# harman097/RoboRugby

Hardware: AMD Instinct MI355X
Metric: env_steps_per_sec (higher is better)
Workload: dtype f64

## Files before the change

roborugby_amd/build.py:

```python
import hashlib
import os
import re
import shutil
import subprocess

HERE = os.path.dirname(os.path.abspath(__file__))
SRC = os.path.join(HERE, "csrc", "rr_kernels.hip")
SRC_KSTEP = os.path.join(HERE, "csrc", "rr_kstep_inst.hip")
SRC_DQN = os.path.join(HERE, "csrc", "rr_dqn.hip")
HDR_KSTEP = os.path.join(HERE, "csrc", "rr_kstep.hpp")
DEPS = [SRC, SRC_KSTEP, SRC_DQN, HDR_KSTEP, os.path.join(HERE, "csrc", "rr_sim.hpp"),
        os.path.join(HERE, "csrc", "rr_extras.hpp"), os.path.join(HERE, "csrc", "rr_hive.hpp"), os.path.join(HERE, "csrc", "rr_render.hpp"),
        os.path.join(os.path.dirname(HERE), "include", "roborugby_amd.h")]
LIB = os.path.join(HERE, "libroborugby_amd.so")
LIB_EXACT = os.path.join(HERE, "libroborugby_amd_exact.so")
HIPCC_FLAGS = ["-O3", "--offload-arch=gfx950", "-std=c++17", "-ffp-contract=off", "-fPIC", "-shared"]


def header_config_rows():
    with open(HDR_KSTEP) as f:
        text = f.read()
    parts = int(re.search(r"^#define RR_KSTEP_PARTS (\d+)$", text, re.M).group(1))
    table = re.search(r"^#else // the product library.*?^#endif", text, re.M | re.S).group(0)
    rows = [tuple(int(v) for v in m.groups()) for m in re.finditer(r"X\((\d+), (\d+), (\d+), (\d+), (\d+), (\d+), \w+, (\d+)\)", table)]
    if not rows or sorted({r[1] for r in rows}) != list(range(parts)):
        raise RuntimeError("csrc/rr_kstep.hpp: the configuration table does not use every part 0..RR_KSTEP_PARTS-1")
    return parts, rows


def header_config_table():
    parts, rows = header_config_rows()
    return parts, {r[2:6] for r in rows}


KSTEP_PARTS = 4
BUILT_SHAPES = {(1, 0, 1, 0), (2, 2, 4, 4), (1, 1, 1, 1)}


def find_hipcc():
    for cand in (shutil.which("hipcc"), "/opt/rocm/bin/hipcc"):
        if cand and os.path.exists(cand):
            return cand
    raise RuntimeError("hipcc not found: the MI355X library cannot be built here")


def sources_present():
    return all(os.path.exists(d) for d in DEPS)


def source_hash():
    h = hashlib.sha256(" ".join(HIPCC_FLAGS).encode())
    for d in DEPS:
        with open(d, "rb") as f:
            h.update(os.path.basename(d).encode() + b"\0" + f.read())
    return h.hexdigest()


def is_stale(exact=False):
    lib = LIB_EXACT if exact else LIB
    if not os.path.exists(lib) or not os.path.exists(lib + ".srchash"):
        return True
    with open(lib + ".srchash") as f:
        return f.read().strip() != source_hash()


def build_hip_library(force=False, verbose=False, jobs=None, exact=False):
    lib_path = LIB_EXACT if exact else LIB
    if not force and not is_stale(exact):
        return lib_path
    import tempfile
    from concurrent.futures import ThreadPoolExecutor
    if header_config_table() != (KSTEP_PARTS, BUILT_SHAPES):
        raise RuntimeError("roborugby_amd/build.py: KSTEP_PARTS / BUILT_SHAPES differ from the table in csrc/rr_kstep.hpp")
    digest = source_hash()
    hipcc = find_hipcc()
    cflags = [f for f in HIPCC_FLAGS if f != "-shared"] + (["-DRR_EXACT_TRIG=1"] if exact else [])
    jobs = jobs or int(os.environ.get("RR_BUILD_JOBS", "0")) or min(8, os.cpu_count() or 1)
    with tempfile.TemporaryDirectory(prefix="rr_build_") as tmpd:
        units = [(SRC, ["-DRR_SPLIT_BUILD"], os.path.join(tmpd, "rr_kernels.o"))]
        units += [(SRC_KSTEP, [f"-DRR_PART={k}"], os.path.join(tmpd, f"rr_kstep_{k}.o")) for k in range(KSTEP_PARTS)]
        units += [(SRC_DQN, [], os.path.join(tmpd, "rr_dqn.o"))]

        def compile_one(u):
            src, defs, obj = u
            cmd = [hipcc] + cflags + defs + ["-c", "-o", obj, src]
            if verbose:
                print(" ".join(cmd), flush=True)
            subprocess.check_call(cmd)
            return obj

        with ThreadPoolExecutor(max_workers=jobs) as ex:
            objs = list(ex.map(compile_one, units))
        tmp = lib_path + f".tmp{os.getpid()}"
        cmd = [hipcc, "--offload-arch=gfx950", "-fPIC", "-shared", "-o", tmp] + objs
# ... 66 lines not shown
```

roborugby_amd/csrc/rr_kernels.hip:

```cpp
#include <hip/hip_runtime.h>
#include <stdio.h>
#include <string.h>
#include <cmath>
#include <new>
#include <string>
#include <type_traits>
#include <cstdlib>

#include "../../include/roborugby_amd.h"
#include "rr_sim.hpp"
#include "rr_extras.hpp"
#include "rr_hive.hpp"
#include "rr_render.hpp"
#include "rr_kstep.hpp"

using namespace rr;


#ifndef RR_ORDER_SHIFT
#define RR_ORDER_SHIFT 2
#endif
constexpr int ORDER_BINS = 1024, ORDER_THREADS = 1024;
__global__ __launch_bounds__(ORDER_THREADS) void k_order(const uint32_t *cost, uint32_t *order, int ngroups) {
    __shared__ uint32_t hist[ORDER_BINS];
    for (int i = threadIdx.x; i < ORDER_BINS; i += ORDER_THREADS) hist[i] = 0;
    __syncthreads();
    for (int g = threadIdx.x; g < ngroups; g += ORDER_THREADS) {
        uint32_t c = cost[g] >> RR_ORDER_SHIFT;
        c = c > ORDER_BINS - 1 ? ORDER_BINS - 1 : c;
        atomicAdd(&hist[ORDER_BINS - 1 - c], 1u);
    }
    __syncthreads();
    __shared__ uint32_t scan[ORDER_BINS];
    uint32_t v = hist[threadIdx.x];
    scan[threadIdx.x] = v;
    __syncthreads();
    for (int off = 1; off < ORDER_BINS; off <<= 1) {
        uint32_t add = threadIdx.x >= (unsigned)off ? scan[threadIdx.x - off] : 0u;
        __syncthreads();
        scan[threadIdx.x] += add;
        __syncthreads();
    }
    hist[threadIdx.x] = scan[threadIdx.x] - v;
    __syncthreads();
    for (int g = threadIdx.x; g < ngroups; g += ORDER_THREADS) {
        uint32_t c = cost[g] >> RR_ORDER_SHIFT;
        c = c > ORDER_BINS - 1 ? ORDER_BINS - 1 : c;
        order[atomicAdd(&hist[ORDER_BINS - 1 - c], 1u)] = (uint32_t)g;
    }
}
__global__ void k_iota(uint32_t *order, int n) {
    int i = blockIdx.x * blockDim.x + threadIdx.x;
    if (i < n) order[i] = (uint32_t)i;
}

template <class C, typename O>
__global__ __launch_bounds__(64 * WAVES_PER_BLOCK) void k_reset(SimParams<typename C::Real> sp, typename C::Store *recs,
                                                               int32_t *irecs, int n, const uint8_t *mask, int init,
                                                               O *obs, O *obs_g) {
    using R = typename C::Real;
    __shared__ Arena<C> lds[arenas_per_block<C>()];
    const int wave = threadIdx.x / C::VW;
    const int arena = blockIdx.x * arenas_per_block<C>() + wave;
    if (arena >= n || wave >= arenas_per_block<C>()) return;
    Arena<C> &A = lds[wave];
    typename C::Store *rec = recs + (size_t)arena * Arena<C>::P_STRIDE;
    int32_t *irec = irecs + (size_t)arena * Arena<C>::I_STRIDE;
    int st = 0;
    if (init) {
        const int lane = threadIdx.x & (C::VW - 1);
        R *p = reinterpret_cast<R *>(&A.p);
        int32_t *q = reinterpret_cast<int32_t *>(&A.i);
        for (int k = lane; k < Arena<C>::P_REALS; k += C::VW) p[k] = (R)0;
        for (int k = lane; k < Arena<C>::I_INTS; k += C::VW) q[k] = 0;
        RR_SYNC();
        if (lane < C::NR) robot_set_clean_lane(A, sp, lane, (R)0, (R)0, lane < C::NRH ? (R)90 : (R)-90);
        if (lane < C::NB) ball_set_clean_lane(A, lane, (R)0, (R)0, (R)0, (R)0);
        if (lane == 0) A.i.episode = -1;
        RR_SYNC();
    } else {
        load_record(A, rec, irec);
    }
    const bool doit = init || !mask || mask[arena];
    if (doit) reset_arena(A, sp, sp.arena_offset + (uint64_t)arena, (uint64_t)(uint32_t)(A.i.episode + 1), st);
    else derive(A, sp);
    if (obs && doit) observe<C, O>(A, sp, 1, -1, -1, obs + (size_t)arena * 11, st);
    if (obs_g && doit) {
        if (!observe<C, O>(A, sp, -1, -1, -1, obs_g + (size_t)arena * 11, st)) {
            for (int k = threadIdx.x & (C::VW - 1); k < 11; k += C::VW) obs_g[(size_t)arena * 11 + k] = (O)NAN;
        }
    }
    store_record(A, rec, irec);
}

template <class C, typename O>
__global__ __launch_bounds__(64 * WAVES_PER_BLOCK) void k_observe(SimParams<typename C::Real> sp, const typename C::Store *recs,
                                                                 const int32_t *irecs, int n, int team, int ridx, int bidx,
                                                                 O *obs) {
    __shared__ Arena<C> lds[arenas_per_block<C>()];
    const int wave = threadIdx.x / C::VW;
    const int arena = blockIdx.x * arenas_per_block<C>() + wave;
    if (arena >= n || wave >= arenas_per_block<C>()) return;
    Arena<C> &A = lds[wave];
    load_record(A, recs + (size_t)arena * Arena<C>::P_STRIDE, irecs + (size_t)arena * Arena<C>::I_STRIDE);
    derive(A, sp);
    int st = 0;
    if (!observe<C, O>(A, sp, team, ridx, bidx, obs + (size_t)arena * 11, st)) {
        for (int k = threadIdx.x & (C::VW - 1); k < 11; k += C::VW) obs[(size_t)arena * 11 + k] = (O)NAN;
    }
}

template <class C>
__global__ void k_set_state(typename C::Store *recs, int32_t *irecs, int n, const double *robots, const int32_t *ri,
                            const double *balls, const int32_t *step) {
    using R = typename C::Real;
    int a = blockIdx.x * blockDim.x + threadIdx.x;
    if (a >= n) return;
    typename C::Store *rec = recs + (size_t)a * Arena<C>::P_STRIDE;
    int32_t *irec = irecs + (size_t)a * Arena<C>::I_STRIDE;
    using L = RecLayout<C>;
    constexpr int NR = C::NR, NB = C::NB;
    for (int r = 0; r < NR; r++) {
        for (int f = 0; f < L::ROBOT_FIELDS; f++) rec[L::robot_field(f) + r] = (typename C::Store)robots[((size_t)a * NR + r) * L::ROBOT_FIELDS + f];
        for (int f = 0; f < 3; f++) irec[L::robot_int(f) + r] = ri[((size_t)a * NR + r) * 3 + f];
    }
    for (int b = 0; b < NB; b++)
        for (int f = 0; f < L::BALL_FIELDS; f++) rec[L::ball_field(f) + b] = (typename C::Store)balls[((size_t)a * NB + b) * L::BALL_FIELDS + f];
    irec[L::STEP] = step[a];
    irec[L::FAULT] = 0;
// ... 158 lines not shown
    __shared__ Arena<C> lds[arenas_per_block<C>()];
    const int wave = threadIdx.x / C::VW;
    const int arena = blockIdx.x * arenas_per_block<C>() + wave;
    if (arena >= n || wave >= arenas_per_block<C>()) return;
    const int32_t *irec = irecs + (size_t)arena * Arena<C>::I_STRIDE;
    if constexpr (HELD) {
        if (hive_hold<C>(irec, held + arena)) return;
    }
    Arena<C> &A = lds[wave];
    const typename C::Store *rec = recs + (size_t)arena * Arena<C>::P_STRIDE;
    load_record(A, rec, irec);
    if (KIND == OBS_V2) derive(A, sp);
    Rec<C> q = { rec };
    hive_observe<C, O, KIND>(A, q, sp, robot_mask, assign + (size_t)arena * C::NR, obs + (size_t)arena * C::NR * 11);
}
__global__ __launch_bounds__(256) void k_hive_commit(int n, int nr, uint32_t robot_mask, const int32_t *fresh, const int32_t *assign,
                                                     const uint8_t *held, int32_t *accepted, float *thrust) {
    const int cell = blockIdx.x * 256 + threadIdx.x;
    if (cell >= n * nr) return;
    const int a = cell / nr, r = cell - a * nr;
    const size_t row = (size_t)a * nr;
    hive_commit(robot_mask, r, fresh + row, assign + row, held[a], accepted + row, thrust + 2 * row);
}
template <class C, typename O, int KIND, bool HELD = false>
__global__ __launch_bounds__(64 * WAVES_PER_BLOCK, lds_waves_per_simd<C>()) void k_hive_transition(
    SimParams<typename C::Real> sp, const typename C::Store *recs, const int32_t *irecs, int n, const typename C::Real *xs, uint32_t robot_mask,
    const int32_t *assign, const int32_t *status, const uint8_t *done, O *next_obs, O *reward, uint8_t *terminal, uint8_t *valid) {
    __shared__ Arena<C> lds[arenas_per_block<C>()];
    const int wave = threadIdx.x / C::VW;
    const int arena = blockIdx.x * arenas_per_block<C>() + wave;
    if (arena >= n || wave >= arenas_per_block<C>()) return;
    const size_t row = (size_t)arena * C::NR;
    if constexpr (HELD) {
        if (hive_idle<C, O>(status[arena], next_obs + row * 11, reward + row, terminal + row, valid + row)) return;
    }
    Arena<C> &A = lds[wave];
    const typename C::Store *rec = recs + (size_t)arena * Arena<C>::P_STRIDE;
    load_record(A, rec, irecs + (size_t)arena * Arena<C>::I_STRIDE);
    if (KIND == OBS_V2) derive(A, sp);
    Rec<C> q = { rec };
    hive_transition<C, O, KIND>(A, q, sp, xs + (size_t)arena * xs_stride<C>(), robot_mask, assign + row, status[arena], done[arena],
                                next_obs + row * 11, reward + row, terminal + row, valid + row);
}

__global__ void k_policy_chase(const float *obs, int n, int na, uint32_t noise_u32, uint64_t seed, uint64_t arena_offset,
                               const int32_t *step_of, uint32_t step, int32_t *actions) {
    const int a = blockIdx.x * blockDim.x + threadIdx.x;
    if (a >= n) return;
    const float d = fmodf(obs[(size_t)a * 11 + 1] - obs[(size_t)a * 11 + 0] + 540.0f, 360.0f) - 180.0f;
    int act = fabsf(d) < 8.0f ? 0 : (d > 0.0f ? 2 : 3);
    const uint64_t gid = arena_offset + (uint64_t)a;
    const uint32_t st = step_of ? (uint32_t)step_of[a] : step;
    uint32_t c[4] = { (uint32_t)gid, (uint32_t)(gid >> 32), st, 0x70C1u };
    philox4x32(c, (uint32_t)seed, (uint32_t)(seed >> 32));
    if (c[0] < noise_u32) act = (int)(c[1] & 7u);
    actions[(size_t)a * na] = act;
    for (int k = 1; k < na; k++) actions[(size_t)a * na + k] = (int)((c[2 + (k & 1)] >> (4 * (k >> 1))) & 7u);
}

typedef unsigned int u32x4 __attribute__((ext_vector_type(4)));
__global__ __launch_bounds__(256) void k_copy16(const u32x4 *__restrict__ src, u32x4 *__restrict__ dst, size_t n16) {
    const size_t i = (size_t)blockIdx.x * 256 + threadIdx.x;
    if (i < n16) dst[i] = src[i];
}

struct rr_env {
    rr_config cfg;
    int kind;
    int vw;
    void *recs;
    int32_t *irecs;
    size_t rec_bytes, irec_bytes;
    uint32_t *snap;
    int32_t *isnap;
    SimParams<double> spd;
    SimParams<float> spf;
    Program prog;
    bool custom_prog;
    bool track_prior;
    int32_t *gs;
    void *xs;
    int32_t *status_buf;
    uint32_t *order;
    uint32_t *cost;
    int ngroups;
    uint32_t *park;
    uint32_t budget;
    int32_t *flag;
};

static thread_local std::string g_err;
static int fail(int code, const std::string &msg) { g_err = msg; return code; }
#define HIP_TRY(expr)                                                                            \
    do {                                                                                         \
        hipError_t e_ = (expr);                                                                  \
        if (e_ != hipSuccess) return fail(-2, std::string(#expr) + ": " + hipGetErrorString(e_)); \
    } while (0)

template <typename R> static void fill_params(SimParams<R> &sp, const rr_config &c) {
    derive_constants(sp, c.arena_w, c.arena_h);
    sp.game_len = c.game_len_steps; sp.game_mode = c.game_mode; sp.time_limit = c.time_limit; sp.auto_reset = c.auto_reset;
    sp.reset_on_fault = c.reset_on_fault;
    sp.acc_external = 0;
    { const char *nm = getenv("RR_NO_MEMO"); sp.memo = (nm && atoi(nm)) ? 0 : 1; }
    sp.seed = c.seed; sp.arena_offset = c.arena_offset;
}
template <typename R> static const SimParams<R> &params_of(const rr_env *e);
template <> const SimParams<double> &params_of<double>(const rr_env *e) { return e->spd; }
template <> const SimParams<float> &params_of<float>(const rr_env *e) { return e->spf; }

template <class F> static int dispatch(const rr_env *e, F &&f) {
#define X(kind_, part_, a, b, c, d, R_, vw_) \
    if (e->kind == kind_) return f(Cfg<a, b, c, d, R_, vw_>{});
    RR_CFG_TABLE(X)
#undef X
    return fail(-1, "corrupt handle");
}
struct DeviceGuard {
    int prev = -1;
    bool switched = false;
    explicit DeviceGuard(int want) {
        if (hipGetDevice(&prev) == hipSuccess && prev != want) switched = (hipSetDevice(want) == hipSuccess);
    }
    ~DeviceGuard() { if (switched) (void)hipSetDevice(prev); }
};

template <class C> struct Typed {
    using Cfg = C;
    using R = typename C::Real;
    const rr_env *e;
    hipStream_t s;
    int n() const { return e->cfg.num_envs; }
    typename C::Store *recs() const { return static_cast<typename C::Store *>(e->recs); }
    int32_t *irecs() const { return e->irecs; }
    R *xs() const { return static_cast<R *>(e->xs); }
    const SimParams<R> &sp() const { return params_of<R>(e); }
    template <class... P, class... A> void per_thread(void (*k)(P...), const A &...a) const {
        hipLaunchKernelGGL(k, dim3((unsigned)((n() + 127) / 128)), dim3(128), 0, s, static_cast<P>(a)...);
    }
    template <class... P, class... A> void per_wave(void (*k)(P...), const A &...a) const {
        hipLaunchKernelGGL(k, dim3((unsigned)((n() + arenas_per_block<C>() - 1) / arenas_per_block<C>())), dim3(64 * WAVES_PER_BLOCK), 0, s,
                           static_cast<P>(a)...);
    }
};
template <typename O = float, class F>
static int on_handle(rr_env *e, const char *who, void *stream, F &&f, const char *f64_refusal = nullptr) {
    if (!e) return fail(-1, std::string(who) + ": null handle");
    DeviceGuard guard(e->cfg.device);
    int rc = dispatch(e, [&](auto c) {
        using C = decltype(c);
        if constexpr (std::is_same<O, double>::value && !std::is_same<typename C::Real, double>::value) return fail(-1, f64_refusal);
        else return f(Typed<C>{ e, (hipStream_t)stream });
    });
    if (rc) return rc;
    HIP_TRY(hipGetLastError());
    return 0;
}

extern "C" {

int rr_abi_version(void) { return RR_ABI_VERSION; }
int rr_exact_trig(void) { return RR_EXACT_TRIG; }
const char *rr_last_error(void) { return g_err.c_str(); }

int rr_create(const rr_config *cfg, rr_env **out) {
    if (!cfg || !out) return fail(-1, "rr_create: null argument");
    if (cfg->struct_size != (int32_t)sizeof(rr_config)) return fail(-1, "rr_create: rr_config.struct_size mismatch");
    if (cfg->num_envs <= 0) return fail(-1, "rr_create: num_envs must be positive");
    int shape = -1;
#define X(kind_, part_, a, b, c, d, R_, vw_) \
    if (shape < 0 && cfg->nr_happy == a && cfg->nr_grumpy == b && cfg->nb_pos == c && cfg->nb_neg == d) shape = kind_ % RR_NUM_SHAPES;
    RR_CFG_TABLE(X)
#undef X
#if defined(RR_CUSTOM_SHAPE)
    if (shape < 0) return fail(-1, "rr_create: this library was built for one shape only (roborugby_amd.build.build_shape_library) and it is not this one");
    if (cfg->dtype == RR_DTYPE_F32) return fail(-1, "rr_create: a one-shape library is built for RR_DTYPE_F64 and RR_DTYPE_F32_STATE only");
#else
    if (shape < 0)
        return fail(-1, "rr_create: unsupported entity counts (built shapes: 1+0 robots/1+0 balls, 2+2 robots/4+4 balls, 1+1 robots/1+1 balls; "
                        "any other counts: a one-shape library, roborugby_amd.build.build_shape_library / BatchedRoboRugbyEnv does it on demand)");
#endif
    if (cfg->dtype != RR_DTYPE_F64 && cfg->dtype != RR_DTYPE_F32 && cfg->dtype != RR_DTYPE_F32_STATE) return fail(-1, "rr_create: bad dtype");
    if (cfg->dtype == RR_DTYPE_F32_STATE && cfg->step_budget_clocks) return fail(-1, "rr_create: no step budget with RR_DTYPE_F32_STATE");
    if (!(cfg->arena_w >= 300 && cfg->arena_h >= 300 && cfg->arena_w <= 8192 && cfg->arena_h <= 8192))
        return fail(-1, "rr_create: arena size out of range [300, 8192]");
    if (cfg->game_len_steps <= 0) return fail(-1, "rr_create: game_len_steps must be positive");
    int ndev = 0;
    HIP_TRY(hipGetDeviceCount(&ndev));
    if (cfg->device < 0 || cfg->device >= ndev) return fail(-1, "rr_create: no such HIP device");
    DeviceGuard guard(cfg->device);
    rr_env *e = new (std::nothrow) rr_env();
    if (!e) return fail(-3, "rr_create: out of host memory");
    e->cfg = *cfg;
    e->kind = shape + RR_NUM_SHAPES * cfg->dtype;
    e->prog.n = 3; e->prog.id[0] = KEEPER_NAUGHTY; e->prog.id[1] = KEEPER_CHASE; e->prog.id[2] = KEEPER_PUSHPOS;
    fill_params(e->spd, *cfg);
    fill_params(e->spf, *cfg);
    size_t pstride = 0, preals = 0, snapw = 0, isnapw = 0;
    int apb = 1;
    const size_t rsz = cfg->dtype == RR_DTYPE_F64 ? 8 : 4;
    dispatch(e, [&](auto c) {
        using CC = decltype(c);
        e->vw = CC::VW;
        pstride = Arena<CC>::P_STRIDE; preals = Arena<CC>::P_REALS; snapw = Arena<CC>::SNAP_WORDS; isnapw = Arena<CC>::ISNAP_WORDS;
        apb = arenas_per_block<CC>();
        return 0;
    });
    const int n = cfg->num_envs;
    e->rec_bytes = pstride * rsz;
    e->irec_bytes = 0;
    hipError_t he = hipMalloc(&e->recs, e->rec_bytes * (size_t)n);
    if (he == hipSuccess && e->spd.memo) {
        he = hipMalloc((void **)&e->snap, 4 * snapw * (size_t)n);
        if (he == hipSuccess) he = hipMalloc((void **)&e->isnap, 4 * isnapw * (size_t)n);
    }
    if (he != hipSuccess) {
        rr_destroy(e);
        return fail(-3, std::string("rr_create: hipMalloc: ") + hipGetErrorString(he));
    }
    e->irecs = reinterpret_cast<int32_t *>(static_cast<char *>(e->recs) + preals * rsz);
    const int ng = (n + apb - 1) / apb;
    const char *no = getenv("RR_NO_ORDER");
    if (ng > 2048 && ng <= 65536 && !(no && atoi(no))) {
        if (hipMalloc((void **)&e->order, sizeof(uint32_t) * ng) == hipSuccess && hipMalloc((void **)&e->cost, sizeof(uint32_t) * ng) == hipSuccess) {
            e->ngroups = ng;
            hipLaunchKernelGGL(k_iota, dim3((ng + 255) / 256), dim3(256), 0, 0, e->order, ng);
            (void)hipMemset(e->cost, 0, sizeof(uint32_t) * ng);
        } else {
            if (e->order) (void)hipFree(e->order);
            e->order = nullptr; e->cost = nullptr;
        }
    }
    dispatch(e, [&](auto c) {
        Typed<decltype(c)> v = { e, nullptr };
        v.per_wave(k_reset<decltype(c), float>, v.sp(), v.recs(), v.irecs(), n, nullptr, 1, nullptr, nullptr);
        return 0;
    });
    he = hipGetLastError();
    if (he == hipSuccess) he = hipDeviceSynchronize();
    if (he != hipSuccess) {
        rr_destroy(e);
        return fail(-2, std::string("rr_create: init kernel: ") + hipGetErrorString(he));
    }
    if (cfg->step_budget_clocks) {
        if (int rc = rr_set_step_budget(e, cfg->step_budget_clocks)) { rr_destroy(e); return rc; }
    }
    *out = e;
    return 0;
}

int rr_destroy(rr_env *e) {
    if (!e) return 0;
    DeviceGuard guard(e->cfg.device);
    for (void *p : { e->recs, (void *)e->snap, (void *)e->isnap, e->xs, (void *)e->gs, (void *)e->status_buf, (void *)e->order, (void *)e->cost,
                     (void *)e->park, (void *)e->flag })
        if (p) (void)hipFree(p);
    delete e;
    return 0;
}

int rr_reset(rr_env *e, const uint8_t *mask, float *obs, float *obs_g, void *stream) {
    return on_handle(e, "rr_reset", stream, [&](auto v) {
        using C = typename decltype(v)::Cfg;
        v.per_wave(k_reset<C, float>, v.sp(), v.recs(), v.irecs(), v.n(), mask, 0, obs, obs_g);
        if (e->track_prior && e->xs)
            v.per_thread(k_extras_begin<C>, v.recs(), v.n(), v.xs(), mask);
        if (e->gs) v.per_thread(k_goal_clear<C>, v.n(), e->gs, mask);
        return 0;
    });
}

static int check_step_args(rr_env *e, const void *act, int32_t na, const void *obs, const void *reward, const void *done) {
    if (!e) return fail(-1, "rr_step: null handle");
    if (!act || !obs || !reward || !done) return fail(-1, "rr_step: actions/obs/reward/done must be non-null");
    const int nr = e->cfg.nr_happy + e->cfg.nr_grumpy;
    if (na < 0 || na > nr)
        return fail(-1, "rr_step: more actions than robots");
    return 0;
}

extern "C++" {
template <typename O>
static int step_impl(rr_env *e, const int32_t *actions, const float *thrust, int32_t na, O *obs, O *reward, uint8_t *done,
                     O *obs_g, O *reward_g, int32_t *status, void *stream, int nsteps = 1, int repeat = 0) {
    if ((e->custom_prog || e->track_prior || e->gs) && !status) status = e->status_buf;
    return on_handle<O>(e, "rr_step", stream, [&](auto v) {
        using C = typename decltype(v)::Cfg;
        const int n = v.n();
        const bool extras = e->custom_prog || e->track_prior;
        auto step = [&](auto kernel, int ns, int rep, uint32_t *park, uint32_t budget) {
            v.per_wave(kernel, v.sp(), v.recs(), v.irecs(), n, actions, thrust, na, obs, reward, done, obs_g, reward_g, status, e->order, e->cost,
                       ns, rep, e->snap, e->isnap, park, budget);
        };
        if (extras) v.per_thread(k_extras_begin<C>, v.recs(), n, v.xs(), nullptr);
        if constexpr (C::MIXED) {
            if (nsteps != 1 || e->park) return fail(-1, "RR_DTYPE_F32_STATE: rr_step only (no rr_rollout, no step budget)");
            step(k_step<C, O, false>, 1, 0, nullptr, 0);
        } else {
            if (nsteps == 1 && e->park) step(k_step<C, O, false, true>, 1, 0, e->park, e->budget);
            else if (nsteps == 1) step(k_step<C, O, false>, 1, 0, nullptr, 0);
            else if constexpr (std::is_same<O, float>::value) step(k_step<C, O, true>, nsteps, repeat, nullptr, 0);
            else return fail(-1, "rr_rollout: float outputs only");
        }
        if (e->order) hipLaunchKernelGGL(k_order, dim3(1), dim3(ORDER_THREADS), 0, v.s, (const uint32_t *)e->cost, e->order, e->ngroups);
        if (extras) v.per_thread(k_extras_end<C, O>, v.sp(), v.recs(), n, v.xs(), e->prog, e->custom_prog ? 1 : 0, reward, reward_g, status, done);
        if (e->gs) {
            int bd = 0;
            for (int k = 0; k < e->prog.n; k++) bd |= e->prog.id[k] == KEEPER_BASEDESTRUCTION;
            v.per_thread(k_goal<C, O>, v.sp(), v.recs(), v.irecs(), n, e->gs, bd, reward, reward_g, done, status);
        }
        return 0;
    }, "fp64 outputs need a handle created with RR_DTYPE_F64");
}
}

int rr_step(rr_env *e, const int32_t *actions, int32_t na, float *obs, float *reward, uint8_t *done, float *obs_g,
            float *reward_g, int32_t *status, void *stream) {
    if (int rc = check_step_args(e, actions, na, obs, reward, done)) return rc;
    return step_impl<float>(e, actions, nullptr, na, obs, reward, done, obs_g, reward_g, status, stream);
}
int rr_rollout(rr_env *e, const int32_t *actions, int32_t na, int32_t nsteps, int32_t repeat, float *obs, float *reward,
               uint8_t *done, float *obs_g, float *reward_g, int32_t *status, void *stream) {
    if (int rc = check_step_args(e, actions, na, obs, reward, done)) return rc;
    if (nsteps < 1 || nsteps > 4096) return fail(-1, "rr_rollout: nsteps must be in 1..4096");
    if (e->custom_prog || e->track_prior || e->gs)
        return fail(-1, "rr_rollout: the side kernels of a custom reward program / prior-step tracking / goal scoring bracket single steps; use rr_step");
    if (e->park) return fail(-1, "rr_rollout: not on a handle that has had a step budget (arenas may be parked mid-step); use rr_step");
    return step_impl<float>(e, actions, nullptr, na, obs, reward, done, obs_g, reward_g, status, stream, (int)nsteps, repeat != 0);
}
int rr_step_thrust(rr_env *e, const float *thrust, int32_t nk, float *obs, float *reward, uint8_t *done, float *obs_g,
                   float *reward_g, int32_t *status, void *stream) {
    if (int rc = check_step_args(e, thrust, nk, obs, reward, done)) return rc;
    return step_impl<float>(e, nullptr, thrust, nk, obs, reward, done, obs_g, reward_g, status, stream);
}
int rr_step_f64(rr_env *e, const int32_t *actions, int32_t na, double *obs, double *reward, uint8_t *done, double *obs_g,
                double *reward_g, int32_t *status, void *stream) {
    if (int rc = check_step_args(e, actions, na, obs, reward, done)) return rc;
    return step_impl<double>(e, actions, nullptr, na, obs, reward, done, obs_g, reward_g, status, stream);
}
int rr_step_thrust_f64(rr_env *e, const float *thrust, int32_t nk, double *obs, double *reward, uint8_t *done, double *obs_g,
                       double *reward_g, int32_t *status, void *stream) {
    if (int rc = check_step_args(e, thrust, nk, obs, reward, done)) return rc;
    return step_impl<double>(e, nullptr, thrust, nk, obs, reward, done, obs_g, reward_g, status, stream);
}

static int ensure_snapshot_buffer(rr_env *e) {
    if (e->xs) return 0;
    size_t bytes = 0;
    dispatch(e, [&](auto c) { using C = decltype(c); bytes = sizeof(typename C::Real) * xs_stride<C>() * (size_t)e->cfg.num_envs; return 0; });
    HIP_TRY(hipMalloc(&e->xs, bytes));
    HIP_TRY(hipMemset(e->xs, 0, bytes));
    return 0;
}
static int ensure_status_buffer(rr_env *e) {
    if (!e->status_buf) HIP_TRY(hipMalloc((void **)&e->status_buf, sizeof(int32_t) * (size_t)e->cfg.num_envs));
    return 0;
}

static int any_parked(rr_env *e, void *stream, bool &parked) {
    parked = false;
    if (!e->park) return 0;
    hipStream_t s = (hipStream_t)stream;
    if (!e->flag) HIP_TRY(hipMalloc((void **)&e->flag, sizeof(int32_t)));
    HIP_TRY(hipMemsetAsync(e->flag, 0, sizeof(int32_t), s));
    if (int rc = on_handle(e, "any_parked", stream, [&](auto v) {
            v.per_thread(k_any_parked<typename decltype(v)::Cfg>, v.irecs(), v.n(), e->flag);
            return 0;
        }))
        return rc;
    int32_t h = 0;
    HIP_TRY(hipMemcpyAsync(&h, e->flag, sizeof(int32_t), hipMemcpyDeviceToHost, s));
    HIP_TRY(hipStreamSynchronize(s));
    parked = h != 0;
    return 0;
}
static int refuse_if_parked_without_copies(rr_env *e, void *stream, const char *who) {
    if (e->custom_prog || e->track_prior || !e->park) return 0;
    bool parked = false;
    if (int rc = any_parked(e, stream, parked)) return rc;
    if (parked)
        return fail(-1, std::string(who) + ": arenas are parked mid-step (budgeted step) and no on_step_begin copies were kept when their "
                                           "step began; rr_set_step_budget(env, 0) and one rr_step complete every parked step first");
    return 0;
}

int rr_set_reward_program(rr_env *e, const int32_t *ids, int32_t n) {
    if (!e || (!ids && n > 0)) return fail(-1, "rr_set_reward_program: null argument");
// ... 377 lines not shown
```

roborugby_amd/csrc/rr_kstep.hpp:

```cpp
#pragma once
#include <hip/hip_runtime.h>
#include <stdint.h>
#include <type_traits>
#include "rr_sim.hpp"

using namespace rr;

template <class C> __device__ __forceinline__ void load_record(Arena<C> &A, const typename C::Store *rec, const int32_t *irec) {
    using R = typename C::Real;
    R *p = reinterpret_cast<R *>(&A.p);
    int32_t *q = reinterpret_cast<int32_t *>(&A.i);
    const int lane = threadIdx.x & (C::VW - 1);
    for (int k = lane; k < Arena<C>::P_REALS; k += C::VW) p[k] = (R)rec[k];
    for (int k = lane; k < Arena<C>::I_INTS; k += C::VW) q[k] = irec[k];
    RR_SYNC();
}
template <class C> __device__ __forceinline__ void store_record(const Arena<C> &A, typename C::Store *rec, int32_t *irec) {
    using R = typename C::Real;
    const R *p = reinterpret_cast<const R *>(&A.p);
    const int32_t *q = reinterpret_cast<const int32_t *>(&A.i);
    const int lane = threadIdx.x & (C::VW - 1);
    RR_SYNC();
    for (int k = lane; k < Arena<C>::P_REALS; k += C::VW) rec[k] = (typename C::Store)p[k];
    constexpr int TAIL = Arena<C>::I_STRIDE - Arena<C>::P_REALS * Arena<C>::WS;
    for (int k = lane; k < TAIL; k += C::VW) irec[k] = k < Arena<C>::I_INTS ? q[k] : 0;
}

#ifndef RR_MIN_WAVES_PER_SIMD
#define RR_MIN_WAVES_PER_SIMD 4
#endif
#ifndef RR_WAVES_PER_BLOCK
#define RR_WAVES_PER_BLOCK 1
#endif
constexpr int WAVES_PER_BLOCK = RR_WAVES_PER_BLOCK;
template <class C> constexpr int arenas_per_block() { return 64 * WAVES_PER_BLOCK / C::VW; }
template <class C> constexpr int lds_waves_per_simd() {
    constexpr int per_cu = (160 * 1024) / (int)(sizeof(Arena<C>) * arenas_per_block<C>()) * WAVES_PER_BLOCK;
    return per_cu / 4 < 1 ? 1 : (per_cu / 4 > RR_MIN_WAVES_PER_SIMD ? RR_MIN_WAVES_PER_SIMD : per_cu / 4);
}


template <class C, typename O, bool MULTI, bool BUDGET = false>
__global__ __launch_bounds__(64 * WAVES_PER_BLOCK, lds_waves_per_simd<C>()) void k_step(SimParams<typename C::Real> sp, typename C::Store *recs,
                                                              int32_t *irecs, int n, const int32_t *actions,
                                                              const float *thrust, int na, O *obs, O *reward,
                                                              uint8_t *done, O *obs_g, O *reward_g, int32_t *status,
                                                              const uint32_t *order, uint32_t *cost, int nsteps, int repeat,
                                                              uint32_t *snap, int32_t *isnap, uint32_t *park = nullptr,
                                                              uint32_t budget = 0) {
    static_assert(!(MULTI && BUDGET), "rr_rollout keeps the record in LDS across steps: no barrier to budget");
    __shared__ Arena<C> lds[arenas_per_block<C>()];
    const int wave = threadIdx.x / C::VW;
    const unsigned long long t_begin = (cost || BUDGET) ? __builtin_amdgcn_s_memtime() : 0ull;
    const int group = order ? (int)order[blockIdx.x] : (int)blockIdx.x;
    const int arena = group * arenas_per_block<C>() + wave;
    if (arena >= n) return;
    Arena<C> &A = lds[wave];
    typename C::Store *rec = recs + (size_t)arena * Arena<C>::P_STRIDE;
    int32_t *irec = irecs + (size_t)arena * Arena<C>::I_STRIDE;
    RR_T0();
#if defined(RR_PROFILE_PHASES)
    const unsigned long long rr_wave_t0_ = __builtin_amdgcn_s_memrealtime();
#endif
    load_record(A, rec, irec);
    derive(A, sp);
    RR_STAMP(12);
    if constexpr (!MULTI) {
        StepOut<O> o = { obs, obs_g, reward, reward_g, done, status, sp.memo ? snap : nullptr, isnap, arena,
                         (int)Arena<C>::SNAP_WORDS, (int)Arena<C>::ISNAP_WORDS };
        if constexpr (BUDGET) {
            ParkCtx pk;
            pk.buf = park + (size_t)arena * Arena<C>::PARK_WORDS; pk.budget = budget; pk.t_begin = t_begin;
            step_arena<C, O, true>(A, sp, sp.arena_offset + (uint64_t)arena, actions ? actions + (size_t)arena * na : nullptr,
                                   thrust ? thrust + (size_t)arena * 2 * na : nullptr, na, o, pk);
        } else {
            step_arena<C, O>(A, sp, sp.arena_offset + (uint64_t)arena, actions ? actions + (size_t)arena * na : nullptr,
                             thrust ? thrust + (size_t)arena * 2 * na : nullptr, na, o);
        }
    } else {
#pragma unroll 1
        for (int s = 0; s < nsteps; s++) {
            const size_t so = (size_t)s * (size_t)n;
            StepOut<O> o = { obs + so * 11, obs_g ? obs_g + so * 11 : nullptr, reward + so, reward_g ? reward_g + so : nullptr, done + so,
                             status ? status + so : nullptr, sp.memo ? snap : nullptr, isnap, arena,
                             (int)Arena<C>::SNAP_WORDS, (int)Arena<C>::ISNAP_WORDS };
            const size_t ao = repeat ? 0 : so;
            step_arena<C, O>(A, sp, sp.arena_offset + (uint64_t)arena, actions ? actions + (ao + (size_t)arena) * na : nullptr,
                             thrust ? thrust + (ao + (size_t)arena) * 2 * na : nullptr, na, o);
        }
    }
    RR_TR();
    {
        int arena_again = arena;
        asm volatile("" : "+v"(arena_again));
        store_record(A, recs + (size_t)arena_again * Arena<C>::P_STRIDE, irecs + (size_t)arena_again * Arena<C>::I_STRIDE);
    }
    RR_STAMP(13);
    if (cost && threadIdx.x == 0) {
        const unsigned long long dt = ((__builtin_amdgcn_s_memtime() - t_begin) >> 8) / (unsigned)(MULTI ? nsteps : 1);
        cost[group] = dt > 0xFFFFull ? 0xFFFFu : (uint32_t)dt;
    }
#if defined(RR_PROFILE_PHASES)
    if ((threadIdx.x & 63) == 0 && blockIdx.x < 65536) {
        g_rr_wave_t[2 * blockIdx.x] = rr_wave_t0_;
        g_rr_wave_t[2 * blockIdx.x + 1] = __builtin_amdgcn_s_memrealtime();
    }
#endif
}

#define RR_KSTEP_PARTS 4
#if defined(RR_CUSTOM_SHAPE)
#define RR_CFG_TABLE(X) X(0, 0, RR_NRH, RR_NRG, RR_NBP, RR_NBN, double, RR_CVW) X(6, 0, RR_NRH, RR_NRG, RR_NBP, RR_NBN, F32State, RR_CVW)
#elif defined(RR_CFG_SUBSET)
#ifndef RR_TUNE_VW_T
#define RR_TUNE_VW_T 2
#endif
#ifndef RR_TUNE_VW_G
#define RR_TUNE_VW_G 8
#endif
#ifdef RR_TUNE_VW_D
#define RR_TUNE_ROW_D(X) X(2, 0, 1, 1, 1, 1, double, RR_TUNE_VW_D)
#else
#define RR_TUNE_ROW_D(X)
#endif
#define RR_CFG_TABLE(X) X(0, 0, 1, 0, 1, 0, double, RR_TUNE_VW_T) X(1, 0, 2, 2, 4, 4, double, RR_TUNE_VW_G) RR_TUNE_ROW_D(X)
#else
#define RR_CFG_TABLE(X)                                                                                                 \
    X(0, 1, 1, 0, 1, 0, double, 2) X(1, 0, 2, 2, 4, 4, double, 8) X(2, 3, 1, 1, 1, 1, double, 4)                         \
    X(3, 0, 1, 0, 1, 0, float, 2) X(4, 1, 2, 2, 4, 4, float, 8) X(5, 2, 1, 1, 1, 1, float, 4)                            \
    X(6, 3, 1, 0, 1, 0, F32State, 2) X(7, 2, 2, 2, 4, 4, F32State, 8) X(8, 2, 1, 1, 1, 1, F32State, 4)
#endif
constexpr int RR_NUM_SHAPES = 3;
#define X(kind_, part_, a, b, c, d, R_, vw_) static_assert(part_ >= 0 && part_ < RR_KSTEP_PARTS && kind_ >= 0 && kind_ < 3 * RR_NUM_SHAPES, "row");
RR_CFG_TABLE(X)
#undef X

#define RR_KSTEP_SIG(C_, O_)                                                                                                       \
    (SimParams<typename C_::Real>, typename C_::Store *, int32_t *, int, const int32_t *, const float *, int, O_ *, O_ *, uint8_t *, \
     O_ *, O_ *, int32_t *, const uint32_t *, uint32_t *, int, int, uint32_t *, int32_t *, uint32_t *, uint32_t)
#define RR_KSTEP_CFG(a, b, c, d, R_, vw_) Cfg<a, b, c, d, R_, vw_>
#define RR_KSTEP_ONE(PREFIX, a, b, c, d, R_, vw_, O_, MULTI_, BUDGET_) \
    PREFIX template __global__ void k_step<Cfg<a, b, c, d, R_, vw_>, O_, MULTI_, BUDGET_> RR_KSTEP_SIG(RR_KSTEP_CFG(a, b, c, d, R_, vw_), O_);
#define RR_KSTEP_PLAIN(PREFIX, a, b, c, d, R_, vw_, O_) RR_KSTEP_ONE(PREFIX, a, b, c, d, R_, vw_, O_, false, false)
#define RR_KSTEP_BUDGET(PREFIX, a, b, c, d, R_, vw_, O_) RR_KSTEP_ONE(PREFIX, a, b, c, d, R_, vw_, O_, false, true)
#define RR_KSTEP_MULTI(PREFIX, a, b, c, d, R_, vw_, O_) RR_KSTEP_ONE(PREFIX, a, b, c, d, R_, vw_, O_, true, false)
#define RR_KSTEP_INST_double(PREFIX, a, b, c, d, vw_)                                                                                   \
    RR_KSTEP_PLAIN(PREFIX, a, b, c, d, double, vw_, float) RR_KSTEP_BUDGET(PREFIX, a, b, c, d, double, vw_, float)                      \
    RR_KSTEP_MULTI(PREFIX, a, b, c, d, double, vw_, float)                                                                              \
    RR_KSTEP_PLAIN(PREFIX, a, b, c, d, double, vw_, double) RR_KSTEP_BUDGET(PREFIX, a, b, c, d, double, vw_, double)
#define RR_KSTEP_INST_float(PREFIX, a, b, c, d, vw_)                                                                                    \
    RR_KSTEP_PLAIN(PREFIX, a, b, c, d, float, vw_, float) RR_KSTEP_BUDGET(PREFIX, a, b, c, d, float, vw_, float)                        \
    RR_KSTEP_MULTI(PREFIX, a, b, c, d, float, vw_, float)
#define RR_KSTEP_INST_F32State(PREFIX, a, b, c, d, vw_) \
    RR_KSTEP_PLAIN(PREFIX, a, b, c, d, F32State, vw_, float) RR_KSTEP_PLAIN(PREFIX, a, b, c, d, F32State, vw_, double)

#if defined(RR_SPLIT_BUILD) && !defined(RR_CFG_SUBSET)
#define X(kind_, part_, a, b, c, d, R_, vw_) RR_KSTEP_INST_##R_(extern, a, b, c, d, vw_)
RR_CFG_TABLE(X)
#undef X
#endif
```

Before: 174.1 million.

## Fold the cost-order sort into the step kernel's extra block with double-buffered order

Adds one extra block to the step launch that, at high priority, builds the next launch's longest-first group order from the cost array with a single-wave histogram sort in LDS. Running groups stamp a 'running' marker with a start time so the sorter can estimate cost for groups that have not finished yet. The order buffer is double-buffered and swapped on the host, which removes the separate single-block k_order launch from the stream. It applies only outside graph capture and only when the scratch fits in LDS. The cost is that the ordering is built from partly stale or estimated costs, and one block sorts instead of simulating.

```diff
diff --git a/roborugby_amd/build.py b/roborugby_amd/build.py
--- a/roborugby_amd/build.py
+++ b/roborugby_amd/build.py
@@ -9,7 +9,7 @@
 SRC_KSTEP = os.path.join(HERE, "csrc", "rr_kstep_inst.hip")
 SRC_DQN = os.path.join(HERE, "csrc", "rr_dqn.hip")
 HDR_KSTEP = os.path.join(HERE, "csrc", "rr_kstep.hpp")
-DEPS = [SRC, SRC_KSTEP, SRC_DQN, HDR_KSTEP, os.path.join(HERE, "csrc", "rr_sim.hpp"),
+DEPS = [SRC, SRC_KSTEP, SRC_DQN, HDR_KSTEP, os.path.join(HERE, "csrc", "rr_sim.hpp"), os.path.join(HERE, "csrc", "rr_order.hpp"),
         os.path.join(HERE, "csrc", "rr_extras.hpp"), os.path.join(HERE, "csrc", "rr_hive.hpp"), os.path.join(HERE, "csrc", "rr_render.hpp"),
         os.path.join(os.path.dirname(HERE), "include", "roborugby_amd.h")]
 LIB = os.path.join(HERE, "libroborugby_amd.so")
diff --git a/roborugby_amd/csrc/rr_kernels.hip b/roborugby_amd/csrc/rr_kernels.hip
--- a/roborugby_amd/csrc/rr_kernels.hip
+++ b/roborugby_amd/csrc/rr_kernels.hip
@@ -26,7 +26,7 @@
     for (int i = threadIdx.x; i < ORDER_BINS; i += ORDER_THREADS) hist[i] = 0;
     __syncthreads();
     for (int g = threadIdx.x; g < ngroups; g += ORDER_THREADS) {
-        uint32_t c = cost[g] >> RR_ORDER_SHIFT;
+        uint32_t c = (cost[g] & COST_MASK) >> RR_ORDER_SHIFT;
         c = c > ORDER_BINS - 1 ? ORDER_BINS - 1 : c;
         atomicAdd(&hist[ORDER_BINS - 1 - c], 1u);
     }
@@ -44,7 +44,7 @@
     hist[threadIdx.x] = scan[threadIdx.x] - v;
     __syncthreads();
     for (int g = threadIdx.x; g < ngroups; g += ORDER_THREADS) {
-        uint32_t c = cost[g] >> RR_ORDER_SHIFT;
+        uint32_t c = (cost[g] & COST_MASK) >> RR_ORDER_SHIFT;
         c = c > ORDER_BINS - 1 ? ORDER_BINS - 1 : c;
         order[atomicAdd(&hist[ORDER_BINS - 1 - c], 1u)] = (uint32_t)g;
     }
@@ -369,6 +369,7 @@
     void *xs;
     int32_t *status_buf;
     uint32_t *order;
+    uint32_t *order_alt;
     uint32_t *cost;
     int ngroups;
     uint32_t *park;
@@ -425,8 +426,9 @@
     template <class... P, class... A> void per_thread(void (*k)(P...), const A &...a) const {
         hipLaunchKernelGGL(k, dim3((unsigned)((n() + 127) / 128)), dim3(128), 0, s, static_cast<P>(a)...);
     }
-    template <class... P, class... A> void per_wave(void (*k)(P...), const A &...a) const {
-        hipLaunchKernelGGL(k, dim3((unsigned)((n() + arenas_per_block<C>() - 1) / arenas_per_block<C>())), dim3(64 * WAVES_PER_BLOCK), 0, s,
+    template <class... P, class... A> void per_wave(void (*k)(P...), const A &...a) const { per_wave_and(0, k, a...); }
+    template <class... P, class... A> void per_wave_and(int more, void (*k)(P...), const A &...a) const {
+        hipLaunchKernelGGL(k, dim3((unsigned)((n() + arenas_per_block<C>() - 1) / arenas_per_block<C>() + more)), dim3(64 * WAVES_PER_BLOCK), 0, s,
                            static_cast<P>(a)...);
     }
 };
@@ -485,12 +487,14 @@
     fill_params(e->spf, *cfg);
     size_t pstride = 0, preals = 0, snapw = 0, isnapw = 0;
     int apb = 1;
+    size_t lds_bytes = 0;
     const size_t rsz = cfg->dtype == RR_DTYPE_F64 ? 8 : 4;
     dispatch(e, [&](auto c) {
         using CC = decltype(c);
         e->vw = CC::VW;
         pstride = Arena<CC>::P_STRIDE; preals = Arena<CC>::P_REALS; snapw = Arena<CC>::SNAP_WORDS; isnapw = Arena<CC>::ISNAP_WORDS;
         apb = arenas_per_block<CC>();
+        lds_bytes = sizeof(Arena<CC>) * arenas_per_block<CC>();
         return 0;
     });
     const int n = cfg->num_envs;
@@ -509,10 +513,14 @@
     const int ng = (n + apb - 1) / apb;
     const char *no = getenv("RR_NO_ORDER");
     if (ng > 2048 && ng <= 65536 && !(no && atoi(no))) {
-        if (hipMalloc((void **)&e->order, sizeof(uint32_t) * ng) == hipSuccess && hipMalloc((void **)&e->cost, sizeof(uint32_t) * ng) == hipSuccess) {
+        const size_t cost_bytes = sizeof(uint32_t) * (size_t)((ng + 3) & ~3);
+        if (hipMalloc((void **)&e->order, sizeof(uint32_t) * ng) == hipSuccess && hipMalloc((void **)&e->cost, cost_bytes) == hipSuccess) {
             e->ngroups = ng;
             hipLaunchKernelGGL(k_iota, dim3((ng + 255) / 256), dim3(256), 0, 0, e->order, ng);
-            (void)hipMemset(e->cost, 0, sizeof(uint32_t) * ng);
+            (void)hipMemset(e->cost, 0, cost_bytes);
+            if (sort_scratch_bytes(ng) <= lds_bytes && hipMalloc((void **)&e->order_alt, sizeof(uint32_t) * ng) == hipSuccess)
+                hipLaunchKernelGGL(k_iota, dim3((ng + 255) / 256), dim3(256), 0, 0, e->order_alt, ng);
+            else e->order_alt = nullptr;
         } else {
             if (e->order) (void)hipFree(e->order);
             e->order = nullptr; e->cost = nullptr;
@@ -539,7 +547,7 @@
 int rr_destroy(rr_env *e) {
     if (!e) return 0;
     DeviceGuard guard(e->cfg.device);
-    for (void *p : { e->recs, (void *)e->snap, (void *)e->isnap, e->xs, (void *)e->gs, (void *)e->status_buf, (void *)e->order, (void *)e->cost,
+    for (void *p : { e->recs, (void *)e->snap, (void *)e->isnap, e->xs, (void *)e->gs, (void *)e->status_buf, (void *)e->order, (void *)e->order_alt, (void *)e->cost,
                      (void *)e->park, (void *)e->flag })
         if (p) (void)hipFree(p);
     delete e;
@@ -575,9 +583,14 @@
         using C = typename decltype(v)::Cfg;
         const int n = v.n();
         const bool extras = e->custom_prog || e->track_prior;
+        uint32_t *order_next = nullptr;
+        if (e->order_alt) {
+            hipStreamCaptureStatus cs = hipStreamCaptureStatusNone;
+            if (hipStreamIsCapturing(v.s, &cs) == hipSuccess && cs == hipStreamCaptureStatusNone) order_next = e->order_alt;
+        }
         auto step = [&](auto kernel, int ns, int rep, uint32_t *park, uint32_t budget) {
-            v.per_wave(kernel, v.sp(), v.recs(), v.irecs(), n, actions, thrust, na, obs, reward, done, obs_g, reward_g, status, e->order, e->cost,
-                       ns, rep, e->snap, e->isnap, park, budget);
+            v.per_wave_and(order_next ? 1 : 0, kernel, v.sp(), v.recs(), v.irecs(), n, actions, thrust, na, obs, reward, done, obs_g, reward_g, status,
+                           e->order, e->cost, ns, rep, e->snap, e->isnap, park, budget, order_next);
         };
         if (extras) v.per_thread(k_extras_begin<C>, v.recs(), n, v.xs(), nullptr);
         if constexpr (C::MIXED) {
@@ -589,7 +602,8 @@
             else if constexpr (std::is_same<O, float>::value) step(k_step<C, O, true>, nsteps, repeat, nullptr, 0);
             else return fail(-1, "rr_rollout: float outputs only");
         }
-        if (e->order) hipLaunchKernelGGL(k_order, dim3(1), dim3(ORDER_THREADS), 0, v.s, (const uint32_t *)e->cost, e->order, e->ngroups);
+        if (order_next) { e->order_alt = e->order; e->order = order_next; }
+        else if (e->order) hipLaunchKernelGGL(k_order, dim3(1), dim3(ORDER_THREADS), 0, v.s, (const uint32_t *)e->cost, e->order, e->ngroups);
         if (extras) v.per_thread(k_extras_end<C, O>, v.sp(), v.recs(), n, v.xs(), e->prog, e->custom_prog ? 1 : 0, reward, reward_g, status, done);
         if (e->gs) {
             int bd = 0;
diff --git a/roborugby_amd/csrc/rr_kstep.hpp b/roborugby_amd/csrc/rr_kstep.hpp
--- a/roborugby_amd/csrc/rr_kstep.hpp
+++ b/roborugby_amd/csrc/rr_kstep.hpp
@@ -3,6 +3,7 @@
 #include <stdint.h>
 #include <type_traits>
 #include "rr_sim.hpp"
+#include "rr_order.hpp"
 
 using namespace rr;
 
@@ -47,10 +48,18 @@
                                                               uint8_t *done, O *obs_g, O *reward_g, int32_t *status,
                                                               const uint32_t *order, uint32_t *cost, int nsteps, int repeat,
                                                               uint32_t *snap, int32_t *isnap, uint32_t *park = nullptr,
-                                                              uint32_t budget = 0) {
+                                                              uint32_t budget = 0, uint32_t *order_next = nullptr) {
     static_assert(!(MULTI && BUDGET), "rr_rollout keeps the record in LDS across steps: no barrier to budget");
     __shared__ Arena<C> lds[arenas_per_block<C>()];
     const int wave = threadIdx.x / C::VW;
+    if (order_next && blockIdx.x == gridDim.x - 1) {
+        static_assert(sizeof(lds) >= sizeof(uint32_t) * (SORT_BINS + SORT_LANES), "the sorter's histogram lives in lds[]");
+        __builtin_amdgcn_s_setprio(3);
+        if (threadIdx.x < SORT_LANES)
+            order_sort_wave(cost, order_next, (int)gridDim.x - 1, __builtin_amdgcn_s_memrealtime(), RR_SORT_SHIFT,
+                            (uint32_t)(MULTI ? nsteps : 1), reinterpret_cast<uint32_t *>(lds));
+        return;
+    }
     const unsigned long long t_begin = (cost || BUDGET) ? __builtin_amdgcn_s_memtime() : 0ull;
     const int group = order ? (int)order[blockIdx.x] : (int)blockIdx.x;
     const int arena = group * arenas_per_block<C>() + wave;
@@ -63,6 +72,8 @@
     const unsigned long long rr_wave_t0_ = __builtin_amdgcn_s_memrealtime();
 #endif
     load_record(A, rec, irec);
+    if (order_next && threadIdx.x == 0)
+        __hip_atomic_store(cost + group, cost_running_word(cost[group], __builtin_amdgcn_s_memrealtime()), __ATOMIC_RELAXED, __HIP_MEMORY_SCOPE_AGENT);
     derive(A, sp);
     RR_STAMP(12);
     if constexpr (!MULTI) {
@@ -90,16 +101,16 @@
         }
     }
     RR_TR();
+    if (cost && threadIdx.x == 0) {
+        const unsigned long long dt = ((__builtin_amdgcn_s_memtime() - t_begin) >> 8) / (unsigned)(MULTI ? nsteps : 1);
+        __hip_atomic_store(cost + group, dt > 0xFFFFull ? 0xFFFFu : (uint32_t)dt, __ATOMIC_RELAXED, __HIP_MEMORY_SCOPE_AGENT);
+    }
     {
         int arena_again = arena;
         asm volatile("" : "+v"(arena_again));
         store_record(A, recs + (size_t)arena_again * Arena<C>::P_STRIDE, irecs + (size_t)arena_again * Arena<C>::I_STRIDE);
     }
     RR_STAMP(13);
-    if (cost && threadIdx.x == 0) {
-        const unsigned long long dt = ((__builtin_amdgcn_s_memtime() - t_begin) >> 8) / (unsigned)(MULTI ? nsteps : 1);
-        cost[group] = dt > 0xFFFFull ? 0xFFFFu : (uint32_t)dt;
-    }
 #if defined(RR_PROFILE_PHASES)
     if ((threadIdx.x & 63) == 0 && blockIdx.x < 65536) {
         g_rr_wave_t[2 * blockIdx.x] = rr_wave_t0_;
@@ -137,7 +148,7 @@
 
 #define RR_KSTEP_SIG(C_, O_)                                                                                                       \
     (SimParams<typename C_::Real>, typename C_::Store *, int32_t *, int, const int32_t *, const float *, int, O_ *, O_ *, uint8_t *, \
-     O_ *, O_ *, int32_t *, const uint32_t *, uint32_t *, int, int, uint32_t *, int32_t *, uint32_t *, uint32_t)
+     O_ *, O_ *, int32_t *, const uint32_t *, uint32_t *, int, int, uint32_t *, int32_t *, uint32_t *, uint32_t, uint32_t *)
 #define RR_KSTEP_CFG(a, b, c, d, R_, vw_) Cfg<a, b, c, d, R_, vw_>
 #define RR_KSTEP_ONE(PREFIX, a, b, c, d, R_, vw_, O_, MULTI_, BUDGET_) \
     PREFIX template __global__ void k_step<Cfg<a, b, c, d, R_, vw_>, O_, MULTI_, BUDGET_> RR_KSTEP_SIG(RR_KSTEP_CFG(a, b, c, d, R_, vw_), O_);
diff --git a/roborugby_amd/csrc/rr_order.hpp b/roborugby_amd/csrc/rr_order.hpp
--- /dev/null
+++ b/roborugby_amd/csrc/rr_order.hpp
@@ -0,0 +1,145 @@
+#pragma once
+#include <stddef.h>
+#include <stdint.h>
+
+#if defined(__HIPCC__)
+#define RR_ORDER_HD __host__ __device__ __forceinline__
+#else
+#define RR_ORDER_HD inline
+#endif
+#if defined(__HIPCC__) && defined(__HIP_DEVICE_COMPILE__)
+#define RR_ORDER_GPU 1
+#else
+#define RR_ORDER_GPU 0
+#endif
+
+namespace rr {
+
+constexpr uint32_t COST_RUNNING = 0x80000000u;
+constexpr uint32_t COST_MASK = 0xFFFFu;
+constexpr uint32_t COST_STAMP_MASK = 0x7FFFu;
+constexpr int COST_STAMP_SHIFT = 4;
+RR_ORDER_HD uint32_t cost_units_of_stamp_units(uint32_t s) { return s + (s >> 1); }
+
+RR_ORDER_HD uint32_t cost_running_word(uint32_t last_word, uint64_t now) {
+    return COST_RUNNING | (((uint32_t)(now >> COST_STAMP_SHIFT) & COST_STAMP_MASK) << 16) | (last_word & COST_MASK);
+}
+RR_ORDER_HD uint32_t cost_key(uint32_t word, uint64_t now, uint32_t per_step = 1) {
+    uint32_t c = word & COST_MASK;
+    if (word & COST_RUNNING) {
+        const uint32_t elapsed = ((uint32_t)(now >> COST_STAMP_SHIFT) - (word >> 16)) & COST_STAMP_MASK;
+        uint32_t run = cost_units_of_stamp_units(elapsed) / per_step;
+        run = run > COST_MASK ? COST_MASK : run;
+        c = run > c ? run : c;
+    }
+    return c;
+}
+
+#ifndef RR_SORT_BINS
+#define RR_SORT_BINS 512
+#endif
+#ifndef RR_SORT_SHIFT
+#define RR_SORT_SHIFT 3
+#endif
+constexpr int SORT_BINS = RR_SORT_BINS, SORT_LANES = 64, SORT_BINS_PER_LANE = SORT_BINS / SORT_LANES, SORT_BATCH = 8;
+static_assert(SORT_BINS % SORT_LANES == 0 && SORT_BINS <= 65536, "a lane owns whole bins; a bin fits the 16-bit stash");
+RR_ORDER_HD uint32_t sort_bin(uint32_t key, int shift) {
+    const uint32_t b = key >> shift;
+    return (uint32_t)(SORT_BINS - 1) - (b > (uint32_t)(SORT_BINS - 1) ? (uint32_t)(SORT_BINS - 1) : b);
+}
+RR_ORDER_HD size_t sort_scratch_bytes(int ng) { return sizeof(uint32_t) * (SORT_BINS + SORT_LANES) + sizeof(uint16_t) * (size_t)((ng + 3) & ~3); }
+
+#if RR_ORDER_GPU
+#define RR_ORDER_FOR_LANES(l) for (int l = (int)(threadIdx.x & (SORT_LANES - 1)), l##_o = 0; l##_o < 1; ++l##_o)
+#define RR_ORDER_SYNC()                                          \
+    do {                                                         \
+        __builtin_amdgcn_fence(__ATOMIC_RELEASE, "wavefront");   \
+        __builtin_amdgcn_wave_barrier();                         \
+        __builtin_amdgcn_fence(__ATOMIC_ACQUIRE, "wavefront");   \
+    } while (0)
+#define RR_ORDER_BUMP(p) atomicAdd((p), 1u)
+#else
+#define RR_ORDER_FOR_LANES(l) for (int l = 0; l < SORT_LANES; ++l)
+#define RR_ORDER_SYNC() do { } while (0)
+#define RR_ORDER_BUMP(p) ((*(p))++)
+#endif
+
+RR_ORDER_HD void order_sort_wave(const uint32_t *cost, uint32_t *order, int ng, uint64_t now, int shift, uint32_t per_step, uint32_t *scratch) {
+    uint32_t *hist = scratch, *part = scratch + SORT_BINS;
+    uint16_t *stash = reinterpret_cast<uint16_t *>(scratch + SORT_BINS + SORT_LANES);
+    const int nquads = (ng + 3) >> 2;
+#if RR_ORDER_GPU
+    __builtin_amdgcn_fence(__ATOMIC_ACQUIRE, "agent");
+#endif
+    RR_ORDER_FOR_LANES(l) {
+        for (int b = l; b < SORT_BINS; b += SORT_LANES) hist[b] = 0;
+    }
+    RR_ORDER_SYNC();
+    RR_ORDER_FOR_LANES(l) {
+        for (int q0 = l; q0 < nquads; q0 += SORT_BATCH * SORT_LANES) {
+            uint32_t w[SORT_BATCH][4];
+#if RR_ORDER_GPU
+#pragma unroll
+#endif
+            for (int j = 0; j < SORT_BATCH; j++) {
+                const int q = q0 + j * SORT_LANES;
+#if RR_ORDER_GPU
+                const uint4 v = q < nquads ? reinterpret_cast<const uint4 *>(cost)[q] : make_uint4(0u, 0u, 0u, 0u);
+                w[j][0] = v.x; w[j][1] = v.y; w[j][2] = v.z; w[j][3] = v.w;
+#else
+                for (int k = 0; k < 4; k++) w[j][k] = q < nquads && 4 * q + k < ng ? cost[4 * q + k] : 0u;
+#endif
+            }
+#if RR_ORDER_GPU
+#pragma unroll
+#endif
+            for (int j = 0; j < SORT_BATCH; j++) {
+                const int q = q0 + j * SORT_LANES;
+                for (int k = 0; k < 4; k++) {
+                    if (4 * q + k >= ng) continue;
+                    const uint32_t b = sort_bin(cost_key(w[j][k], now, per_step), shift);
+                    stash[4 * q + k] = (uint16_t)b;
+                    RR_ORDER_BUMP(&hist[b]);
+                }
+            }
+        }
+    }
+    RR_ORDER_SYNC();
+    RR_ORDER_FOR_LANES(l) {
+        uint32_t s = 0;
+        for (int k = 0; k < SORT_BINS_PER_LANE; k++) s += hist[l * SORT_BINS_PER_LANE + k];
+        part[l] = s;
+    }
+    RR_ORDER_SYNC();
+    RR_ORDER_FOR_LANES(l) {
+        uint32_t base = 0;
+        for (int k = 0; k < SORT_LANES; k++) base += k < l ? part[k] : 0u;
+        for (int k = 0; k < SORT_BINS_PER_LANE; k++) {
+            const uint32_t c = hist[l * SORT_BINS_PER_LANE + k];
+            hist[l * SORT_BINS_PER_LANE + k] = base;
+            base += c;
+        }
+    }
+    RR_ORDER_SYNC();
+    RR_ORDER_FOR_LANES(l) {
+        for (int g0 = l; g0 < ng; g0 += SORT_BATCH * SORT_LANES) {
+            uint32_t pos[SORT_BATCH];
+#if RR_ORDER_GPU
+#pragma unroll
+#endif
+            for (int j = 0; j < SORT_BATCH; j++) {
+                const int g = g0 + j * SORT_LANES;
+                pos[j] = g < ng ? RR_ORDER_BUMP(&hist[stash[g]]) : 0u;
+            }
+#if RR_ORDER_GPU
+#pragma unroll
+#endif
+            for (int j = 0; j < SORT_BATCH; j++) {
+                const int g = g0 + j * SORT_LANES;
+                if (g < ng) order[pos[j]] = (uint32_t)g;
+            }
+        }
+    }
+}
+
+}
```

Result: no change. 175.7 million (median of 6 runs) (+1.0%).
